# djordjijeK/DynamicGraphRepresentationLearning

Measured on AMD Instinct MI355X. Metric: MH walk-steps/sec, higher is better.
Workload: dtype u32

## Files before the change

dynamicgraphrepresentationlearning_amd/csrc/wharf_api.hip:

```cpp
#include <algorithm>
#include <cmath>
#include <cstring>

#include <rocprim/device/device_radix_sort.hpp>
#include <rocprim/device/device_scan.hpp>
#include <rocprim/device/device_segmented_radix_sort.hpp>
#include <rocprim/device/device_select.hpp>
#include <rocprim/iterator/counting_iterator.hpp>

#include <charconv>
#include <unistd.h>
#include <chrono>
#include <stdexcept>
#include <string>
#include <vector>

#include "wharf_gpu.h"
#include "wharf_kernels.h"

using namespace wharf;

namespace {

thread_local std::string g_last_error;
// ... 43 lines not shown
    }
    void release()
    {
        if (p) (void)hipFree(p);
        p = nullptr;
        cap = 0;
    }
    template <class T> T* as() const { return reinterpret_cast<T*>(p); }
};

uint32_t bits_for(uint64_t x)
{
    uint32_t b = 0;
    while (b < 64 && (x - 1) >> b) b++;
    return b;
}

}

struct wharf_handle {
    int device = 0;
    hipStream_t s = nullptr;
    hipEvent_t ev[6] = {};
    wharf_config cfg{};
    uint64_t n = 0, m = 0, lo = 0, hi = 0, n_loc = 0, W = 0;
    uint32_t sh_part = 0, sh_parts = 1, sh_bits = 0;

    ShardMap smap() const { return ShardMap{n, n_loc, lo, sh_part, sh_parts, sh_bits}; }
    bool owned_li(uint64_t wid, uint64_t& li) const
    {
        const uint64_t r = wid / n, v = wid % n;
        if (r >= wpv || v < lo || v >= hi) return false;
        const uint64_t off = v - lo, q = off >> sh_bits;
        if (q % sh_parts != sh_part) return false;
        li = r * n_loc + (((q / sh_parts) << sh_bits) | (off & ((1ull << sh_bits) - 1)));
        return true;
    }
    uint32_t L = 0, wpv = 0;
    bool anchors = false, has_walks = false;
    bool walks_poisoned = false;
    void check_walks() const
    {
        REQUIRE(!walks_poisoned, WHARF_E_STATE,
                "the walks are incomplete after a failed update (WHARF_E_STATE); call wharf_generate");
    }
    bool anchors_cold = true;
// ... 560 lines not shown
        a.ehash = anchors ? ehash.as<uint64_t>() : nullptr;
        a.ehash_mask = ehash_mask;
        a.fdir = anchors && fpool.p ? fdir.as<uint64_t>() : nullptr;
        a.fpool = anchors && fpool.p ? fpool.as<uint32_t>() : nullptr;
        a.walks = walks.as<uint32_t>();
        a.rtab = rtab.as<uint64_t>();
        a.bitmap = bitmap.as<uint32_t>();
        a.bloom = bitmap.as<uint32_t>() + bitmap_words();
        a.aff = aff.as<uint8_t>();
        a.counters = counters.as<unsigned long long>();
        a.n = n; a.n_loc = n_loc; a.lo = lo; a.W = W; a.wpv = wpv;
        a.sh_part = sh_part; a.sh_parts = sh_parts; a.sh_bits = sh_bits;
        a.L = L; a.epoch = epoch;
        a.key0 = (uint32_t)cfg.seed; a.key1 = (uint32_t)(cfg.seed >> 32);
        a.inv_p = 1.0f / cfg.paramP;
        a.inv_q = 1.0f / cfg.paramQ;
        a.model = cfg.model; a.init = cfg.sampler_init; a.det = cfg.deterministic;
        const char* ns = getenv("WHARF_NO_SURE_SKIP");
        a.no_sure = ns && atoi(ns) ? 1 : 0;
        const char* ls = getenv("WHARF_N2V_LANE_SORT");
        a.lane_sort = ls && *ls ? (atoi(ls) != 0) : 1;
        a.err = errflag.as<unsigned long long>() + 5;
        a.stage = 0;
        const char* rf = getenv("WHARF_RET_FIRST");
        a.ret_first = cfg.model == WHARF_NODE2VEC && !cfg.deterministic && cfg.sampler_init == WHARF_INIT_WEIGHT &&
                      !a.no_sure && a.inv_q != 1.0f && a.inv_p > fmaxf(1.0f, a.inv_q) && rf && *rf && atoi(rf) != 0;
        return a;
    }

    float elapsed(int a, int b)
    {
        float ms = 0;
        HIPCHK(hipEventElapsedTime(&ms, ev[a], ev[b]));
        return ms;
    }

    void read_counters()
    {
        unsigned long long c[8] = {};
        HIPCHK(hipMemcpyAsync(c, counters.p, 64, hipMemcpyDeviceToHost, s));
        sync();
        st.steps = c[0];
        st.accepts = c[1];
        st.last_anchor_inits = c[7];
        st.last_rewalk_passes = st_park_passes;
#ifdef WHARF_INIT_STATS
// ... 26 lines not shown
    try {
        if (h) HIPCHK(hipSetDevice(h->device));
        f();
        return WHARF_OK;
    } catch (const WharfError& e) {
        set_err(h, e.what());
        return e.code;
    } catch (const std::exception& e) {
        set_err(h, e.what());
        return WHARF_E_INVALID;
    }
}

void check_config(const wharf_config* c)
{
    REQUIRE(c, WHARF_E_INVALID, "config is null");
    REQUIRE(c->walks_per_vertex >= 1 && c->walks_per_vertex <= 255, WHARF_E_INVALID, "walks_per_vertex must be 1..255");
    REQUIRE(c->walk_length >= 2 && c->walk_length <= 255, WHARF_E_INVALID, "walk_length must be 2..255 (types::Position is u8)");
    REQUIRE(c->model == WHARF_DEEPWALK || c->model == WHARF_NODE2VEC, WHARF_E_INVALID, "Unrecognized random walking model");
    REQUIRE(c->sampler_init >= WHARF_INIT_RANDOM && c->sampler_init <= WHARF_INIT_WEIGHT, WHARF_E_INVALID,
            "Unrecognized sampler init strategy");
    REQUIRE(c->model != WHARF_NODE2VEC || (c->paramP > 0 && c->paramQ > 0), WHARF_E_INVALID, "paramP/paramQ must be > 0");
}

wharf_handle* new_handle(const wharf_config* cfg, uint64_t n, int device)
{
    check_config(cfg);
    REQUIRE(n >= 1 && n < 0xFFFFFFFEull, WHARF_E_INVALID, "n must be in [1, 2^32-2)");
    REQUIRE(n * (uint64_t)cfg->walks_per_vertex < (1ull << 32), WHARF_E_INVALID,
            "n * walks_per_vertex must be < 2^32 (types::WalkID is u32)");
    int ndev = 0;
    HIPCHK(hipGetDeviceCount(&ndev));
    REQUIRE(device >= 0 && device < ndev, WHARF_E_INVALID, "no such HIP device " + std::to_string(device));
    HIPCHK(hipSetDevice(device));
    auto* h = new wharf_handle();
    h->device = device;
    h->cfg = *cfg;
    h->n = n;
    h->L = cfg->walk_length;
    h->wpv = cfg->walks_per_vertex;
    h->lo = cfg->shard_lo;
    h->hi = cfg->shard_hi ? cfg->shard_hi : n;
    if (h->lo > h->hi || h->hi > n) {
        delete h;
        throw WharfError(WHARF_E_INVALID, "shard range must satisfy shard_lo <= shard_hi <= n");
    }
    h->n_loc = h->hi - h->lo;
    h->W = h->n_loc * h->wpv;
    h->anchors = cfg->model == WHARF_NODE2VEC && !cfg->deterministic;
    HIPCHK(hipStreamCreateWithFlags(&h->s, hipStreamNonBlocking));
    for (auto& e : h->ev) HIPCHK(hipEventCreate(&e));
    std::vector<uint64_t> t((size_t)h->wpv * h->L);
    for (uint32_t r = 0; r < h->wpv; r++) {
        XoroHost x(r);
        for (uint32_t j = 0; j < h->L; j++) t[(size_t)r * h->L + j] = x.lrand();
    }
    h->rtab.ensure(t.size() * 8);
    HIPCHK(hipMemcpy(h->rtab.p, t.data(), t.size() * 8, hipMemcpyHostToDevice));
    h->counters.ensure(64);
    h->errflag.ensure(64);
    return h;
}

void free_handle(wharf_handle* h)
{
    if (!h) return;
    (void)hipSetDevice(h->device);
    if (h->s) (void)hipStreamSynchronize(h->s);
    for (DevBuf* b : {&h->off, &h->adj, &h->deg, &h->cap, &h->vrec, &h->erec, &h->erec2, &h->ehash, &h->fdir, &h->fpool,
                      &h->fplan, &h->memo, &h->srcidx, &h->row_epoch, &h->off2, &h->adj2, &h->walks, &h->aff, &h->rtab,
                      &h->bitmap, &h->counters, &h->errflag, &h->tmp, &h->k1, &h->k2, &h->flags, &h->chg, &h->cf,
                      &h->runstart, &h->runs, &h->count, &h->pairs, &h->sel, &h->defer, &h->rplan, &h->pscan,
                      &h->scratch, &h->stab, &h->preoff, &h->park, &h->parkc, &h->bdesc, &h->sanc, &h->rchunk,
                      &h->rev, &h->srev, &h->sg_counts, &h->sg_noise, &h->sg_ids, &h->sg_cols, &h->sg_stat,
                      &h->sg_out})
        b->release();
    h->free_snaps();
    for (auto& e : h->ev)
        if (e) (void)hipEventDestroy(e);
    if (h->s) (void)hipStreamDestroy(h->s);
    delete h;
}

void build_graph_from_keys(wharf_handle* h, uint64_t cnt, bool drop_loops, bool symmetric_by_construction)
{
    const uint64_t mm = h->unique_keys(cnt, drop_loops, 32 + std::max<uint32_t>(bits_for(h->n), 1));
    h->symmetric = symmetric_by_construction;
    h->csr_from_keys(mm);
    const char* rv = getenv("WHARF_REV");
    const bool rev_may = rv && *rv ? atoi(rv) != 0 : h->pool_cap >= wharf_handle::kRevMinPool;
    if (!symmetric_by_construction && (h->anchors || rev_may)) {
        unsigned long long* asym = h->errflag.as<unsigned long long>() + 3;
        HIPCHK(hipMemsetAsync(asym, 0, 8, h->s));
        launch_keys_symmetric(h->k1.as<uint64_t>(), mm, asym, h->s);
        unsigned long long v = 1;
        HIPCHK(hipMemcpyAsync(&v, asym, 8, hipMemcpyDeviceToHost, h->s));
        h->sync();
        h->symmetric = v == 0;
    }
    for (DevBuf* b : {&h->k1, &h->k2, &h->tmp, &h->flags}) b->release();
    h->finish_graph();
}
// ... 28 lines not shown
    if (!listn) return;
    h->park.ensure(2 * listn * kParkRecBytes);
    h->parkc.ensure(16);
    unsigned long long* pc = h->parkc.as<unsigned long long>();
    char* P[2] = {h->park.as<char>(), h->park.as<char>() + listn * kParkRecBytes};
    HIPCHK(hipMemsetAsync(pc, 0, 16, s));
    launch_rewalk_park(a, 1, 1, nullptr, nullptr, P[0], pc, s);
    const char* te = getenv("WHARF_PARK_TAIL");
    const uint64_t tail = te ? strtoull(te, nullptr, 10) : kParkTail;
    uint32_t passes = 1;
    for (int cur = 0;; cur ^= 1) {
        uint64_t cnt = 0;
        HIPCHK(hipMemcpyAsync(&cnt, pc + cur, 8, hipMemcpyDeviceToHost, s));
        h->sync();
        if (!cnt) break;
        launch_park_init(a, P[cur], pc + cur, s);
        const bool last = cnt < tail;
        HIPCHK(hipMemsetAsync(pc + (cur ^ 1), 0, 8, s));
        launch_rewalk_park(a, 0, last ? 0 : 1, P[cur], pc + cur, P[cur ^ 1], pc + (cur ^ 1), s);
        passes++;
        if (last) break;
    }
    h->st_park_passes = passes;
}

void walk_update(wharf_handle* h, uint64_t k, uint32_t flags, uint32_t* affected_out, uint64_t* n_affected)
{
    hipStream_t s = h->s;
    if (h->has_walks && h->W) {
        HIPCHK(hipMemsetAsync(h->counters.p, 0, 24, s));
        HIPCHK(hipMemsetAsync(h->counters.as<unsigned long long>() + 7, 0, 8, s));
        h->st_park_passes = 0;
        const char* sat = getenv("WHARF_BLOOM_SATURATE");
        if (sat && atoi(sat)) HIPCHK(hipMemsetAsync(h->bitmap.as<uint32_t>() + h->bitmap_words(), 0xFF, kFilterWords * 4, s));
        WalkArgs a = h->walk_args();
        a.scan_only = (flags & WHARF_APPLY_WALK_UPDATES) ? 0 : 1;
        const char* ntr = getenv("WHARF_NT_ROWS");
        a.nt_rows = ntr ? (atoi(ntr) != 0) : ((double)k * h->L >= 0.08 * (double)std::max<uint64_t>(h->n, 1));
        const uint64_t stride4 = (h->L + 3) & ~3ull;
        const char* no_memo = getenv("WHARF_NO_MEMO");
        if (a.det && !a.scan_only && k && !(no_memo && atoi(no_memo)) &&
            (uint64_t)h->wpv * k * stride4 * 4 <= (256ull << 20)) {
            h->srcidx.ensure(std::max<uint64_t>(h->n, 1) * 4);
            h->memo.ensure(((uint64_t)h->wpv * k * stride4 + 2 * kMemoPad) * 4);
            const char* cbm = getenv("WHARF_COPY_BITMAP");
            a.src_exact = !(cbm && atoi(cbm));
// ... 55 lines not shown
        const bool corrupt = n2v_list && lbad && atoi(lbad) != 0;
        if (gsort || corrupt) {
            a.stage = 1;
            launch_walk(a, true, s);
            uint64_t c2 = 0;
            HIPCHK(hipMemcpyAsync(&c2, a.counters + 2, 8, hipMemcpyDeviceToHost, s));
            h->sync();
            const uint64_t cnt = c2 & kListMask;
            REQUIRE(cnt <= h->W, WHARF_E_STATE, "re-walk list longer than the walks");
            if (gsort && cnt > 1) {
                h->park.ensure(cnt * 8);
                uint64_t* in = h->defer.as<uint64_t>();
                uint64_t* out = h->park.as<uint64_t>();
                h->rp([&](void* t, size_t& b) { return rocprim::radix_sort_keys(t, b, in, out, (size_t)cnt, 0u, 64u, s); });
                HIPCHK(hipMemcpyAsync(in, out, cnt * 8, hipMemcpyDeviceToDevice, s));
            }
            if (corrupt && cnt) {
                const uint64_t bad = (h->W + 12345) | (1ull << 56);
                HIPCHK(hipMemcpyAsync(h->defer.as<uint64_t>() + cnt / 2, &bad, 8, hipMemcpyHostToDevice, s));
                h->sync();
            }
            a.stage = 2;
        }
        launch_walk(a, true, s);
        HIPCHK(hipGetLastError());
        if (a.park) park_passes(h, a);
        HIPCHK(hipEventRecord(h->ev[3], s));
        const unsigned nb = aff_blocks(h->W);
        h->sel.ensure((uint64_t)(nb + 1) * 8);
        uint32_t* bcount = h->sel.as<uint32_t>();
        uint32_t* boff = bcount + nb + 1;
        HIPCHK(hipMemsetAsync(bcount + nb, 0, 4, s));
        launch_aff_count(h->aff.as<uint8_t>(), h->W, bcount, s);
        h->rp([&](void* t, size_t& b) {
            return rocprim::exclusive_scan(t, b, bcount, boff, 0u, (size_t)nb + 1, rocprim::plus<uint32_t>(), s);
        });
        const bool on_device = affected_out && (flags & WHARF_AFFECTED_DEVICE);
        if (!on_device) h->pairs.ensure(h->W * 4);
        launch_aff_write(h->aff.as<uint8_t>(), h->W, boff, h->smap(),
                         on_device ? affected_out : h->pairs.as<uint32_t>(), s);
        uint32_t naff32 = 0;
        unsigned long long lerr = 0;
        HIPCHK(hipMemcpyAsync(&naff32, boff + nb, 4, hipMemcpyDeviceToHost, s));
        HIPCHK(hipMemcpyAsync(&lerr, a.err, 8, hipMemcpyDeviceToHost, s));
        h->sync();
        if (lerr) h->walks_poisoned = true;
        REQUIRE(lerr == 0, WHARF_E_STATE,
                std::string("node2vec re-walk list: ") + ((lerr & 1) ? "an entry outside the walks" : "an entry outside its block") +
                    " was skipped; the walks of this update are incomplete");
        const uint64_t naff = naff32;
        if (affected_out && !on_device && naff) {
            HIPCHK(hipMemcpyAsync(affected_out, h->pairs.p, naff * 4, hipMemcpyDeviceToHost, s));
            h->sync();
        }
        h->last_aff.clear();
        h->last_aff_version = ~0ull;
        if (!on_device && naff && naff <= wharf_handle::kStageMax) {
            if (affected_out) {
                h->last_aff.assign(affected_out, affected_out + naff);
            } else {
                h->last_aff.resize(naff);
                HIPCHK(hipMemcpyAsync(h->last_aff.data(), h->pairs.p, naff * 4, hipMemcpyDeviceToHost, s));
                h->sync();
            }
            h->last_aff_version = h->walks_version;
        }
        h->st.affected = naff;
        if (n_affected) *n_affected = naff;
        h->read_counters();
        h->st.last_walk_kernel_ms = h->elapsed(2, 3);
        h->st.last_walk_update_ms = h->elapsed(1, 3);
    } else {
        h->sync();
    }
// ... 1158 lines not shown
```

dynamicgraphrepresentationlearning_amd/csrc/wharf_kernels.h:

```cpp
#pragma once

#include <hip/hip_runtime.h>
#include <stdint.h>

#include <algorithm>

#include "wharf_device.h"

namespace wharf {

enum { kDeepWalk = 0, kNode2Vec = 1 };
enum { kInitRandom = 0, kInitBurnin = 1, kInitWeight = 2 };
constexpr uint64_t kMemoPad = 64;

struct RunInfo {
    uint64_t off, end;
    uint32_t src, rs, re, pad;
};

struct WalkArgs {
    const ERec* vrec;
    const ERec* erec;
    RecFmt rf;
    const uint32_t* deg;
// ... 15 lines not shown
    uint32_t key0, key1;
    float inv_p, inv_q;
    int model, init, det;
    int scan_only;
    uint64_t* defer;
    uint64_t* bdesc;
    uint64_t* stab;
    uint64_t stab_mask;
    uint32_t* memo;
    const uint32_t* src_idx;
    const RunInfo* runs;
    uint64_t memo_k;
    uint32_t memo_stride;
    uint32_t wpv;
    int nt_rows;
    int park;
    int no_sure;
    int lane_sort;
    int src_exact;
    int ret_first;
    unsigned long long* err;
    int stage;
    int plan_group;
};

__host__ __device__ __forceinline__ ShardMap shard_map(const WalkArgs& a)
{
    return ShardMap{a.n, a.n_loc, a.lo, a.sh_part, a.sh_parts, a.sh_bits};
}

constexpr uint64_t kListMask = (1ull << 40) - 1;
constexpr uint64_t kParkRecBytes = 32;


constexpr uint64_t kRelocate = ~0ull;
struct RowPlan {
    uint64_t noff;
    uint32_t ndeg, ncap;
    uint32_t ocap, pad;
};

unsigned grid_for(uint64_t work, unsigned block);
unsigned cu_count();

void launch_walk(const WalkArgs& a, bool rewalk, hipStream_t s);
void launch_rewalk_park(const WalkArgs& a, int fresh, int park, const void* in, const unsigned long long* in_cnt,
// ... 64 lines not shown
                      hipStream_t s);
void launch_patch_in_edges(const uint32_t* adj, uint64_t slots, const uint32_t* bitmap, const uint32_t* bloom,
                           const ERec* vrec, ERec* erec, uint32_t rs, RecFmt rf, hipStream_t s);
constexpr uint32_t kNoRidx = 0xFFFFFFFFu;
void launch_rev_build(const uint64_t* off, const uint32_t* deg, const uint32_t* adj, uint64_t n, uint64_t slots,
                      uint32_t* ridx, unsigned long long* miss, hipStream_t s);
void launch_patch_rev(const RunInfo* runs, uint64_t k, const uint32_t* pre, const uint64_t* off, const uint32_t* deg,
                      const uint32_t* adj, const uint32_t* bitmap, const ERec* vrec, ERec* erec, uint32_t rs,
                      RecFmt rf, uint32_t* ridx, unsigned long long* miss, hipStream_t s);
void launch_transpose(const uint32_t* in, uint64_t W, uint32_t L, uint32_t* out, hipStream_t s);
void launch_gather_rows(const uint32_t* walks, uint64_t W, uint32_t L, const uint64_t* list, uint64_t base,
                        uint64_t count, uint32_t* out, hipStream_t s);
void launch_walk_lengths(const uint32_t* walks, uint64_t W, uint32_t L, uint32_t v0, uint32_t v1, uint64_t* len,
                         hipStream_t s);
void launch_index_entries(const uint32_t* walks, uint64_t W, uint32_t L, const ShardMap& sm, int kb,
                          uint32_t v0, uint32_t v1, const uint64_t* col_base, uint64_t* skeys, uint32_t* vals,
                          hipStream_t s);
void launch_index_split(const uint64_t* skeys, uint64_t E, int kb, unsigned long long* counts, uint64_t* keys,
                        hipStream_t s);
unsigned aff_blocks(uint64_t W);
void launch_aff_count(const uint8_t* aff, uint64_t W, uint32_t* counts, hipStream_t s);
void launch_aff_write(const uint8_t* aff, uint64_t W, const uint32_t* offs, const ShardMap& sm,
                      uint32_t* out, hipStream_t s);
void launch_index_pair(const uint64_t* keys, const uint32_t* nexts, uint64_t E, uint64_t* out, hipStream_t s);
void launch_rel_offsets(const uint64_t* off, uint64_t v0, uint64_t cnt, uint32_t* rel, hipStream_t s);
void launch_fill_u32(uint32_t* p, uint64_t cnt, uint32_t v, hipStream_t s);
void launch_fill_u64(uint64_t* p, uint64_t cnt, uint64_t v, hipStream_t s);
void launch_edge_hash_update(const uint64_t* bkeys, uint64_t mb, const uint32_t* chg, int insert, uint64_t* table,
                             uint64_t mask, hipStream_t s);
void launch_edge_hash_build(const uint64_t* off, const uint32_t* deg, uint64_t n, const uint32_t* adj, uint64_t* table,
                            uint64_t mask, hipStream_t s);
void launch_filter_sizes(const uint32_t* deg, uint64_t n, uint64_t* words, hipStream_t s);
void launch_filter_pack(const uint32_t* deg, uint64_t n, uint64_t* fdir, hipStream_t s);
void launch_filter_fill(const uint64_t* off, const uint32_t* deg, uint64_t n, const uint32_t* adj, const uint64_t* fdir,
                        uint32_t* pool, hipStream_t s);
void launch_filter_plan(const RunInfo* runs, uint64_t k, const uint32_t* deg, const uint64_t* fdir, uint64_t* need,
                        hipStream_t s);
void launch_filter_rows(const RunInfo* runs, uint64_t k, const uint32_t* pre, const uint64_t* noff, const uint32_t* deg,
                        const uint32_t* adj, const uint64_t* need, const uint64_t* gofs, uint64_t base, uint64_t* fdir,
                        uint32_t* pool, hipStream_t s);
void launch_szudzik64(int op, uint64_t cnt, uint64_t* x, uint64_t* y, uint64_t* z, hipStream_t s);

constexpr uint32_t kSgnsNone = 0xFFFFFFFFu;
constexpr uint32_t kSgnsMaxTargets = 16;
constexpr uint32_t kSgnsMaxWindow = 16;
constexpr uint64_t kSgnsSerialCap = 1ull << 20;
// ... 23 lines not shown
```

dynamicgraphrepresentationlearning_amd/csrc/wharf_kernels.hip:

```cpp
#include <cstdlib>
#include <string>
#include <type_traits>

#include "wharf_kernels.h"

namespace wharf {

__device__ __forceinline__ void wave_add(unsigned long long* dst, uint32_t v)
{
#pragma unroll
    for (int o = 32; o > 0; o >>= 1) v += __shfl_xor(v, o, 64);
    if ((threadIdx.x & 63) == 0 && v) atomicAdd(dst, (unsigned long long)v);
}

__device__ __forceinline__ int64_t row_find(const uint32_t* __restrict__ adj, const Row& r, uint32_t x)
{
    uint64_t lo = r.off, hi = r.off + r.deg;
    while (lo < hi) {
        const uint64_t mid = lo + ((hi - lo) >> 1);
        if (adj[mid] < x) lo = mid + 1; else hi = mid;
    }
    return (lo < r.off + r.deg && adj[lo] == x) ? (int64_t)lo : -1;
}

// ... 647 lines not shown
            steps++;
        }
        for (pos = pos + 1; pos < a.L; pos++) walks[(uint64_t)pos * W + li] = kSent;
    }
    wave_add(a.counters + 0, steps);
    wave_add(a.counters + 1, accepts);
    wave_add(a.counters + 7, inits);
}

enum : uint32_t { kLaneScan = 0, kLaneWalk = 1, kLaneDone = 2 };

__device__ __forceinline__ void bloom_to_lds(const WalkArgs& a, uint32_t* s_bloom)
{
    for (uint32_t i = threadIdx.x; i < kBloomWords; i += blockDim.x) s_bloom[i] = a.bloom[i];
    __syncthreads();
}

__device__ __forceinline__ bool is_source(const WalkArgs& a, const uint32_t* s_bloom, uint32_t x)
{
    if (!bloom_test(s_bloom, x)) return false;
    return (a.bitmap[x >> 5] >> (x & 31)) & 1u;
}

template <int MODEL, bool DET, bool BLK = false, int RL = -1>
__global__ __launch_bounds__(256) void k_rewalk_sweep(WalkArgs a)
{
    __shared__ uint32_t s_bloom[kBloomWords];
    bloom_to_lds(a, s_bloom);
    uint32_t steps = 0, accepts = 0, inits = 0;
    const uint64_t stride = (uint64_t)gridDim.x * blockDim.x;
    uint32_t* __restrict__ walks = a.walks;
    const uint64_t W = a.W;
    const uint32_t L = a.L;
    for (uint64_t li = (uint64_t)blockIdx.x * blockDim.x + threadIdx.x; li < W; li += stride) {
        const uint64_t r = li / a.n_loc;
        const uint32_t v = BLK ? walks[li] : start_vertex<false>(a, li - r * a.n_loc);
        const uint64_t wid = r * a.n + v;
        const uint32_t ep = a.epoch << 4, wlo = (uint32_t)wid, whi = (uint32_t)(wid >> 32);
        const uint64_t* __restrict__ rt = DET ? a.rtab + r * L : nullptr;
        uint32_t mode = kLaneScan, p = kNoRewalk;
        uint32_t x = v, xprev = v;
        uint32_t xn = L > 1 ? walks[W + li] : kSent;
        Walker w;
        w.rc.deg = 0;
        for (uint32_t pos = 0; pos < L; pos++) {
            uint32_t val = kSent;
            bool fresh = false;
            if (mode == kLaneWalk) {
                if (w.rc.deg) {
                    val = walk_step<MODEL, DET, false, false, RL>(a, w, rt, DET ? pos - 1 - p : pos - 1, wlo, whi, ep,
                                                                  accepts, inits);
                    steps++;
                }
                fresh = true;
            } else if (mode == kLaneScan) {
                if (pos > 0) {
                    xprev = x;
// ... 186 lines not shown
        if ((a.bitmap[v >> 5] >> (v & 31)) & 1u) return j;
    }
#endif
    ended = t.end < cnt;
    return kScanChunk;
}

__device__ __forceinline__ uint64_t uniform64(uint64_t x)
{
    const uint32_t lo = __builtin_amdgcn_readfirstlane((uint32_t)x), hi = __builtin_amdgcn_readfirstlane((uint32_t)(x >> 32));
    return ((uint64_t)hi << 32) | lo;
}

struct XcdRange {
    uint64_t first, end, stride;
};
__device__ __forceinline__ XcdRange xcd_range(uint64_t W)
{
    const uint32_t xcd = blockIdx.x % kXcds, slot = blockIdx.x / kXcds, per = gridDim.x / kXcds;
    const uint64_t part = (((W + kXcds - 1) / kXcds) + 255) & ~255ull;
    const uint64_t c0 = min(W, (uint64_t)xcd * part);
    return {c0 + (uint64_t)slot * blockDim.x + threadIdx.x, min(W, c0 + part), (uint64_t)per * blockDim.x};
}

#ifndef WHARF_SCAN_WAVES_EU
#define WHARF_SCAN_WAVES_EU 0
#endif
#if WHARF_SCAN_WAVES_EU
#define WHARF_SCAN_WAVES __attribute__((amdgpu_waves_per_eu(WHARF_SCAN_WAVES_EU, WHARF_SCAN_WAVES_EU)))
#else
#define WHARF_SCAN_WAVES
#endif

#ifndef WHARF_SCAN_ONLY_WAVES_EU
#define WHARF_SCAN_ONLY_WAVES_EU 8
#endif
#ifndef WHARF_COPY_EARLY_ROWS
#define WHARF_COPY_EARLY_ROWS 0
#endif
#ifndef WHARF_COPY_WAVES
#define WHARF_COPY_WAVES 1
#endif
template <bool COPY, bool NTL, int FB = 0, bool IDX = false>
__global__ __launch_bounds__(256, COPY ? WHARF_COPY_WAVES : WHARF_SCAN_ONLY_WAVES_EU) WHARF_SCAN_WAVES void k_rewalk_chunked(WalkArgs a)
{
    constexpr uint32_t C = kScanChunk;
    __shared__ uint32_t s_bloom[kBloomWords << FB];
    filter_to_lds<FB>(a, s_bloom);
    uint32_t steps = 0;
    uint32_t* __restrict__ walks = a.walks;
    const uint64_t W = a.W;
    const uint32_t L = a.L;
    const XcdRange xr = xcd_range(W);
    const uint32_t lane = __lane_id();
    for (uint64_t li = xr.first; li < xr.end; li += xr.stride) {
        const uint64_t r = li / a.n_loc;
        uint32_t p = kNoRewalk;
        bool scanning = true;
        const uint32_t* __restrict__ row = nullptr;
        uint32_t* __restrict__ wb = walks + uniform64(li - lane);
        uint32_t cur[C], nxt[C];
#pragma unroll
        for (uint32_t j = 0; j < C; j++) cur[j] = j < L ? row_load<NTL>(wb + (uint64_t)j * W, lane) : kSent;
        for (uint32_t c0 = 0; c0 < L; c0 += C) {
            const uint32_t cnt = min(C, L - c0);
            const bool was_scanning = scanning;
            const bool more = c0 + C < L;
            ChunkTest ct;
            if (scanning) chunk_issue<FB, WHARF_CHUNK_LEAN != 0, COPY && IDX>(a, s_bloom, cur, cnt, ct);
            if ((!COPY || WHARF_COPY_EARLY_ROWS) && more && scanning) {
#pragma unroll
                for (uint32_t j = 0; j < C; j++)
                    nxt[j] = c0 + C + j < L ? row_load<NTL>(wb + (uint64_t)(c0 + C + j) * W, lane) : kSent;
            }
            if (scanning) {
                bool ended = false;
// ... 717 lines not shown
static unsigned walk_grid(uint64_t W)
{
    static int per_cu = -1;
    if (per_cu < 0) {
        const char* e = getenv("WHARF_WALK_BLOCKS_PER_CU");
        per_cu = e ? std::max(0, atoi(e)) : 0;
    }
    const uint64_t full = (W + 255) / 256;
    if (per_cu <= 0) return (unsigned)full;
    return (unsigned)std::min<uint64_t>(full, (uint64_t)cu_count() * per_cu);
}

static unsigned list_grid() { return cu_count() * 8; }

static bool flat_list()
{
    const char* e = getenv("WHARF_N2V_REWALK");
    return e && std::string(e) == "flat";
}

void launch_walk(const WalkArgs& a, bool rewalk, hipStream_t s)
{
    if (a.W == 0) return;
    const dim3 grid(rewalk ? std::min<uint64_t>((a.W + 255) / 256, (uint64_t)cu_count() * 8) : walk_grid(a.W)),
        block(256);
    const dim3 lgrid(list_grid());
    const char* pk = getenv("WHARF_PLAN_KERNEL");
    const bool plan_lean = !(pk && std::string(pk) == "chunked") && a.W <= kLeanMaxW;
    const dim3 pgrid((unsigned)std::min<uint64_t>((a.W + 1023) / 1024, (uint64_t)cu_count() * 2));
    const dim3 bgrid((std::max<unsigned>(std::min<uint64_t>((a.W + 1023) / 1024, (uint64_t)cu_count() * 2), kXcds) /
                      kXcds) * kXcds);
    const char* ps = getenv("WHARF_PLAN_SPLIT");
    const bool plan_split = ps && *ps && atoi(ps) != 0;
    const bool cr = a.rf.compact != 0;
#define WHARF_LAUNCH(M, D)                                                                   \
    do {                                                                                     \
        if (rewalk && M == kNode2Vec) {                                                      \
            if (a.stage == 2) {                                                              \
            } else if (plan_lean && plan_split) {                                            \
                if (a.nt_rows) hipLaunchKernelGGL((k_rewalk_scan_lean<true>), bgrid, dim3(1024), 0, s, a); \
                else hipLaunchKernelGGL((k_rewalk_scan_lean<false>), bgrid, dim3(1024), 0, s, a); \
                hipLaunchKernelGGL((k_rewalk_plan_lean<false, true>), pgrid, dim3(1024), 0, s, a); \
            } else if (plan_lean) {                                                          \
                if (a.nt_rows) hipLaunchKernelGGL(k_rewalk_plan_lean<true>, pgrid, dim3(1024), 0, s, a); \
                else hipLaunchKernelGGL(k_rewalk_plan_lean<false>, pgrid, dim3(1024), 0, s, a);  \
            } else {                                                                         \
                hipLaunchKernelGGL(k_rewalk_plan, grid, block, 0, s, a);                     \
            }                                                                                \
              \
            if (!a.scan_only && !a.park && a.stage != 1) {                                   \
                if (a.bdesc) hipLaunchKernelGGL((k_rewalk_block<M>), lgrid, block, 0, s, a);     \
                else if (flat_list()) hipLaunchKernelGGL((k_rewalk_list<M, D>), lgrid, block, 0, s, a); \
                else if (a.ret_first) hipLaunchKernelGGL((k_rewalk_sorted<M, D, M == kNode2Vec>), lgrid, block, 0, s, a); \
                else hipLaunchKernelGGL((k_rewalk_sorted<M, D>), lgrid, block, 0, s, a);     \
            }                                                                                \
        } else if (rewalk) {                                                                 \
            if (cr && a.sh_parts > 1) hipLaunchKernelGGL((k_rewalk_sweep<M, D, true, 1>), grid, block, 0, s, a); \
            else if (cr) hipLaunchKernelGGL((k_rewalk_sweep<M, D, false, 1>), grid, block, 0, s, a); \
            else if (a.sh_parts > 1) hipLaunchKernelGGL((k_rewalk_sweep<M, D, true, 0>), grid, block, 0, s, a); \
            else hipLaunchKernelGGL((k_rewalk_sweep<M, D, false, 0>), grid, block, 0, s, a);     \
        } else {                                                                             \
            if (cr && a.sh_parts > 1) hipLaunchKernelGGL((k_walk<M, D, true, 1>), grid, block, 0, s, a); \
            else if (cr) hipLaunchKernelGGL((k_walk<M, D, false, 1>), grid, block, 0, s, a); \
            else if (a.sh_parts > 1) hipLaunchKernelGGL((k_walk<M, D, true, 0>), grid, block, 0, s, a); \
            else hipLaunchKernelGGL((k_walk<M, D, false, 0>), grid, block, 0, s, a);         \
        }                                                                                    \
    } while (0)
    const dim3 mgrid((std::max<unsigned>(grid.x, kXcds) / kXcds) * kXcds);
    const char* nc = getenv("WHARF_NO_CHUNKED_SCAN");
    const bool chunked = !(nc && atoi(nc));
    if (rewalk && a.det && a.memo && !a.scan_only) {
        hipLaunchKernelGGL(k_det_suffix, grid_for((uint64_t)a.wpv * a.memo_k, 256), 256, 0, s, a);
        const char* cb = getenv("WHARF_COPY_SMALL_BLOOM");
        if (cb && atoi(cb) && a.src_exact) {
            if (a.nt_rows) hipLaunchKernelGGL((k_rewalk_chunked<true, true, 0, true>), mgrid, block, 0, s, a);
            else hipLaunchKernelGGL((k_rewalk_chunked<true, false, 0, true>), mgrid, block, 0, s, a);
        } else if (cb && atoi(cb)) {
            if (a.nt_rows) hipLaunchKernelGGL((k_rewalk_chunked<true, true, 0>), mgrid, block, 0, s, a);
            else hipLaunchKernelGGL((k_rewalk_chunked<true, false, 0>), mgrid, block, 0, s, a);
        } else if (a.src_exact) {
            if (a.nt_rows) hipLaunchKernelGGL((k_rewalk_chunked<true, true, 1, true>), mgrid, block, 0, s, a);
            else hipLaunchKernelGGL((k_rewalk_chunked<true, false, 1, true>), mgrid, block, 0, s, a);
        } else {
            if (a.nt_rows) hipLaunchKernelGGL((k_rewalk_chunked<true, true, 1>), mgrid, block, 0, s, a);
            else hipLaunchKernelGGL((k_rewalk_chunked<true, false, 1>), mgrid, block, 0, s, a);
        }
        return;
    }
    if (rewalk && a.scan_only && chunked) {
        const char* sb = getenv("WHARF_SCAN_SMALL_BLOOM");
        const char* sk = getenv("WHARF_SCAN_KERNEL");
        const bool small = sb && atoi(sb), big = sk && std::string(sk) == "big";
        if (!small && !big && a.W <= kLeanMaxW) {
            if (a.nt_rows) hipLaunchKernelGGL((k_rewalk_scan_lean<true>), bgrid, dim3(1024), 0, s, a);
            else hipLaunchKernelGGL((k_rewalk_scan_lean<false>), bgrid, dim3(1024), 0, s, a);
            return;
        }
        if (!small) {
            if (a.nt_rows) hipLaunchKernelGGL((k_rewalk_scan_big<true>), bgrid, dim3(1024), 0, s, a);
            else hipLaunchKernelGGL((k_rewalk_scan_big<false>), bgrid, dim3(1024), 0, s, a);
            return;
        }
        if (a.nt_rows) hipLaunchKernelGGL((k_rewalk_chunked<false, true>), mgrid, block, 0, s, a);
        else hipLaunchKernelGGL((k_rewalk_chunked<false, false>), mgrid, block, 0, s, a);
        return;
    }
    if (a.det) WHARF_LAUNCH(kDeepWalk, true);
    else if (a.model == kDeepWalk) WHARF_LAUNCH(kDeepWalk, false);
    else WHARF_LAUNCH(kNode2Vec, false);
// ... 926 lines not shown
        keys[i] = k & mask;
        atomicAdd(counts + (k >> kb), 1ull);
    }
}

constexpr uint32_t kAffPerThread = 16, kAffPerBlock = 256 * kAffPerThread;

__device__ __forceinline__ uint32_t aff_count16(const uint8_t* __restrict__ aff, uint64_t W, uint64_t base)
{
    uint32_t c = 0;
    if (base + kAffPerThread <= W) {
        const uint4 q = *reinterpret_cast<const uint4*>(aff + base);
        const uint32_t w[4] = {q.x, q.y, q.z, q.w};
#pragma unroll
        for (int k = 0; k < 4; k++)
#pragma unroll
            for (int b = 0; b < 4; b++) c += ((w[k] >> (8 * b)) & 0xFFu) != kNoRewalk;
    } else {
        for (uint64_t i = base; i < W; i++) c += aff[i] != kNoRewalk;
    }
    return c;
}

__global__ __launch_bounds__(256) void k_aff_count(const uint8_t* __restrict__ aff, uint64_t W, uint32_t* __restrict__ counts)
{
    const uint64_t base = (uint64_t)blockIdx.x * kAffPerBlock + (uint64_t)threadIdx.x * kAffPerThread;
    uint32_t c = base < W ? aff_count16(aff, W, base) : 0;
#pragma unroll
    for (int o = 32; o > 0; o >>= 1) c += __shfl_xor(c, o, 64);
    __shared__ uint32_t part[4];
    if ((threadIdx.x & 63) == 0) part[threadIdx.x >> 6] = c;
    __syncthreads();
    if (threadIdx.x == 0) counts[blockIdx.x] = part[0] + part[1] + part[2] + part[3];
}

__global__ __launch_bounds__(256) void k_aff_write(const uint8_t* __restrict__ aff, uint64_t W, const uint32_t* __restrict__ offs,
                                                   ShardMap sm, uint32_t* __restrict__ out)
{
    const uint64_t base = (uint64_t)blockIdx.x * kAffPerBlock + (uint64_t)threadIdx.x * kAffPerThread;
    const uint32_t c = base < W ? aff_count16(aff, W, base) : 0;
    const uint32_t lane = threadIdx.x & 63, wv = threadIdx.x >> 6;
    uint32_t x = c;
#pragma unroll
    for (int o = 1; o < 64; o <<= 1) {
        const uint32_t y = __shfl_up(x, o, 64);
        if (lane >= (uint32_t)o) x += y;
    }
    __shared__ uint32_t part[4];
    if (lane == 63) part[wv] = x;
    __syncthreads();
    uint32_t pre = x - c;
    for (uint32_t k = 0; k < wv; k++) pre += part[k];
    uint64_t at = (uint64_t)offs[blockIdx.x] + pre;
    if (!c) return;
    const uint64_t end = base + kAffPerThread < W ? base + kAffPerThread : W;
    for (uint64_t l = base; l < end; l++) {
        if (aff[l] == kNoRewalk) continue;
        out[at++] = (uint32_t)sm.wid(l);
    }
}

unsigned aff_blocks(uint64_t W) { return (unsigned)((W + kAffPerBlock - 1) / kAffPerBlock); }
void launch_aff_count(const uint8_t* aff, uint64_t W, uint32_t* counts, hipStream_t s)
{ if (W) hipLaunchKernelGGL(k_aff_count, aff_blocks(W), 256, 0, s, aff, W, counts); }
void launch_aff_write(const uint8_t* aff, uint64_t W, const uint32_t* offs, const ShardMap& sm, uint32_t* out,
                      hipStream_t s)
{ if (W) hipLaunchKernelGGL(k_aff_write, aff_blocks(W), 256, 0, s, aff, W, offs, sm, out); }

__global__ void k_fill_u64(uint64_t* __restrict__ p, uint64_t cnt, uint64_t v)
{
    for (uint64_t i = (uint64_t)blockIdx.x * blockDim.x + threadIdx.x; i < cnt; i += (uint64_t)gridDim.x * blockDim.x)
        p[i] = v;
}

__global__ void k_fill_u32(uint32_t* __restrict__ p, uint64_t cnt, uint32_t v)
{
    for (uint64_t i = (uint64_t)blockIdx.x * blockDim.x + threadIdx.x; i < cnt; i += (uint64_t)gridDim.x * blockDim.x)
        p[i] = v;
}

__device__ __forceinline__ uint64_t isqrt64(uint64_t z)
{
    uint64_t s = (uint64_t)sqrt((double)z);
    while (s * s > z) s--;
    while ((s + 1) * (s + 1) <= z && (s + 1) < 0x100000000ull) s++;
    return s;
}

__global__ void k_szudzik64(int op, uint64_t cnt, uint64_t* __restrict__ x, uint64_t* __restrict__ y, uint64_t* __restrict__ z)
{
// ... 241 lines not shown
```

dynamicgraphrepresentationlearning_amd/distributed.py:

```python
from __future__ import annotations

import os
from dataclasses import dataclass

import numpy as np


class RankFailure(RuntimeError):

    def __init__(self, rank: int, phase: str, message: str):
        super().__init__(f"rank {rank} failed in {phase}: {message}")
        self.rank = rank
        self.phase = phase
        self.message = message


def _dist_active(group=None) -> bool:
    import torch.distributed as dist
    return dist.is_available() and dist.is_initialized()


def agree(err, phase: str, group=None, device="cpu"):
    if not _dist_active(group):
        if err is not None:
# ... 246 lines not shown

    total = torch.zeros((), dtype=torch.int64, device=rows.device)
    pos = torch.arange(L, dtype=torch.int64, device=rows.device)
    for r0 in range(0, rows.shape[0], block_rows):
        blk = rows[r0:r0 + block_rows]
        ids = torch.arange(global_first + r0, global_first + r0 + blk.shape[0], dtype=torch.int64, device=rows.device)
        h = (ids[:, None] * L + pos[None, :]) * _K1
        h = (h ^ (h >> 31)) * _K2
        total += (((blk.to(torch.int64) & 0xFFFFFFFF) + 1) * h).sum()
    return total


def local_corpus_checksum(read_local, shard, n: int, wpv: int, L: int, rows_per_call: int, device="cpu"):
    import torch

    own = shard_size(shard) * wpv
    buf = torch.empty((max(1, min(rows_per_call, own)), L), dtype=torch.int32, device=device)
    total = torch.zeros((), dtype=torch.int64, device=device)
    for f in range(0, own, buf.shape[0]):
        k = min(buf.shape[0], own - f)
        read_local(f, k, buf[:k])
        for lf, c, gf in shard_rows_to_global(shard, n, f, k):
            total += corpus_checksum(buf[lf - f:lf - f + c], gf, L)
    return total
```

Measured before the change: 50.56 billion.

## Slice walk update to overlap affected-id D2H copies with re-walking

```diff
diff --git a/dynamicgraphrepresentationlearning_amd/csrc/wharf_api.hip b/dynamicgraphrepresentationlearning_amd/csrc/wharf_api.hip
--- a/dynamicgraphrepresentationlearning_amd/csrc/wharf_api.hip
+++ b/dynamicgraphrepresentationlearning_amd/csrc/wharf_api.hip
@@ -89,6 +89,10 @@
     int device = 0;
     hipStream_t s = nullptr;
     hipEvent_t ev[6] = {};
+    static constexpr uint32_t kMaxAffSlices = 64;
+    hipStream_t s2 = nullptr;
+    hipEvent_t sev[kMaxAffSlices] = {};
+    uint32_t* slice_cnt = nullptr;
     wharf_config cfg{};
     uint64_t n = 0, m = 0, lo = 0, hi = 0, n_loc = 0, W = 0;
     uint32_t sh_part = 0, sh_parts = 1, sh_bits = 0;
@@ -695,6 +699,7 @@
         a.lane_sort = ls && *ls ? (atoi(ls) != 0) : 1;
         a.err = errflag.as<unsigned long long>() + 5;
         a.stage = 0;
+        a.w_first = 0; a.w_end = W;
         const char* rf = getenv("WHARF_RET_FIRST");
         a.ret_first = cfg.model == WHARF_NODE2VEC && !cfg.deterministic && cfg.sampler_init == WHARF_INIT_WEIGHT &&
                       !a.no_sure && a.inv_q != 1.0f && a.inv_p > fmaxf(1.0f, a.inv_q) && rf && *rf && atoi(rf) != 0;
@@ -767,6 +772,8 @@
             "Unrecognized sampler init strategy");
     REQUIRE(c->model != WHARF_NODE2VEC || (c->paramP > 0 && c->paramQ > 0), WHARF_E_INVALID, "paramP/paramQ must be > 0");
 }
+
+void free_handle(wharf_handle* h);
 
 wharf_handle* new_handle(const wharf_config* cfg, uint64_t n, int device)
 {
@@ -793,17 +800,25 @@
     h->n_loc = h->hi - h->lo;
     h->W = h->n_loc * h->wpv;
     h->anchors = cfg->model == WHARF_NODE2VEC && !cfg->deterministic;
-    HIPCHK(hipStreamCreateWithFlags(&h->s, hipStreamNonBlocking));
-    for (auto& e : h->ev) HIPCHK(hipEventCreate(&e));
-    std::vector<uint64_t> t((size_t)h->wpv * h->L);
-    for (uint32_t r = 0; r < h->wpv; r++) {
-        XoroHost x(r);
-        for (uint32_t j = 0; j < h->L; j++) t[(size_t)r * h->L + j] = x.lrand();
-    }
-    h->rtab.ensure(t.size() * 8);
-    HIPCHK(hipMemcpy(h->rtab.p, t.data(), t.size() * 8, hipMemcpyHostToDevice));
-    h->counters.ensure(64);
-    h->errflag.ensure(64);
+    try {
+        HIPCHK(hipStreamCreateWithFlags(&h->s, hipStreamNonBlocking));
+        for (auto& e : h->ev) HIPCHK(hipEventCreate(&e));
+        HIPCHK(hipStreamCreateWithFlags(&h->s2, hipStreamNonBlocking));
+        for (auto& e : h->sev) HIPCHK(hipEventCreateWithFlags(&e, hipEventDisableTiming));
+        HIPCHK(hipHostMalloc((void**)&h->slice_cnt, wharf_handle::kMaxAffSlices * sizeof(uint32_t), hipHostMallocDefault));
+        std::vector<uint64_t> t((size_t)h->wpv * h->L);
+        for (uint32_t r = 0; r < h->wpv; r++) {
+            XoroHost x(r);
+            for (uint32_t j = 0; j < h->L; j++) t[(size_t)r * h->L + j] = x.lrand();
+        }
+        h->rtab.ensure(t.size() * 8);
+        HIPCHK(hipMemcpy(h->rtab.p, t.data(), t.size() * 8, hipMemcpyHostToDevice));
+        h->counters.ensure(64);
+        h->errflag.ensure(64);
+    } catch (...) {
+        free_handle(h);
+        throw;
+    }
     return h;
 }
 
@@ -812,6 +827,7 @@
     if (!h) return;
     (void)hipSetDevice(h->device);
     if (h->s) (void)hipStreamSynchronize(h->s);
+    if (h->s2) (void)hipStreamSynchronize(h->s2);
     for (DevBuf* b : {&h->off, &h->adj, &h->deg, &h->cap, &h->vrec, &h->erec, &h->erec2, &h->ehash, &h->fdir, &h->fpool,
                       &h->fplan, &h->memo, &h->srcidx, &h->row_epoch, &h->off2, &h->adj2, &h->walks, &h->aff, &h->rtab,
                       &h->bitmap, &h->counters, &h->errflag, &h->tmp, &h->k1, &h->k2, &h->flags, &h->chg, &h->cf,
@@ -823,6 +839,10 @@
     h->free_snaps();
     for (auto& e : h->ev)
         if (e) (void)hipEventDestroy(e);
+    for (auto& e : h->sev)
+        if (e) (void)hipEventDestroy(e);
+    if (h->slice_cnt) (void)hipHostFree(h->slice_cnt);
+    if (h->s2) (void)hipStreamDestroy(h->s2);
     if (h->s) (void)hipStreamDestroy(h->s);
     delete h;
 }
@@ -897,6 +917,85 @@
         if (last) break;
     }
     h->st_park_passes = passes;
+}
+
+constexpr uint64_t kAffSlicesDefault = 8;
+constexpr uint64_t kSliceRounds = 4;
+
+uint64_t slice_blocks(const wharf_handle* h, const WalkArgs& a, uint32_t flags, const uint32_t* affected_out)
+{
+    if (!affected_out || (flags & WHARF_AFFECTED_DEVICE) || a.scan_only) return 0;
+    if (!a.det && a.model != kDeepWalk) return 0;
+    const char* ks = getenv("WHARF_AFF_SLICES");
+    uint64_t K = ks && *ks ? strtoull(ks, nullptr, 10) : kAffSlicesDefault;
+    K = std::min<uint64_t>(K, wharf_handle::kMaxAffSlices);
+    uint64_t min_walks = kSliceRounds * cu_count() * 8 * 256;
+    const char* mw = getenv("WHARF_AFF_SLICE_MIN_WALKS");
+    if (mw && *mw) min_walks = std::max<uint64_t>(strtoull(mw, nullptr, 10), 1);
+    const uint64_t blocks = (h->W + 255) / 256;
+    K = std::min(K, std::min(blocks, h->W / min_walks));
+    if (K < 2) return 0;
+    hipPointerAttribute_t at{};
+    if (hipPointerGetAttributes(&at, affected_out) != hipSuccess) {
+        (void)hipGetLastError();
+        return 0;
+    }
+    if (at.type != hipMemoryTypeHost) return 0;
+    return (blocks + K - 1) / K;
+}
+
+uint64_t walk_update_sliced(wharf_handle* h, WalkArgs a, uint64_t per_blocks, uint32_t* affected_out)
+{
+    hipStream_t s = h->s, s2 = h->s2;
+    const uint64_t W = h->W, per = per_blocks * 256, nsl = (W + per - 1) / per;
+    REQUIRE(nsl <= wharf_handle::kMaxAffSlices, WHARF_E_STATE, "too many slices of the walks");
+    const char* lg = getenv("WHARF_LOG_SLICES");
+    if (lg && atoi(lg))
+        fprintf(stderr, "[wharf] walk update: %llu slices of %llu walks\n", (unsigned long long)nsl, (unsigned long long)per);
+    const uint64_t slot = (uint64_t)aff_blocks(per) + 1;
+    h->sel.ensure(nsl * slot * 8);
+    h->pairs.ensure(W * 4);
+    uint32_t* sel = h->sel.as<uint32_t>();
+    uint32_t* ids = h->pairs.as<uint32_t>();
+    uint64_t naff = 0;
+    try {
+        HIPCHK(hipMemsetAsync(sel, 0, nsl * slot * 8, s));
+        for (uint64_t k = 0; k < nsl; k++) {
+            a.w_first = k * per;
+            a.w_end = std::min(W, a.w_first + per);
+            launch_walk(a, true, s);
+            if (k + 1 == nsl) {
+                HIPCHK(hipGetLastError());
+                HIPCHK(hipEventRecord(h->ev[3], s));
+            }
+            const unsigned nb = aff_blocks(a.w_end - a.w_first);
+            uint32_t* bcount = sel + 2 * k * slot;
+            uint32_t* boff = bcount + slot;
+            launch_aff_count(h->aff.as<uint8_t>(), a.w_first, a.w_end, bcount, s);
+            h->rp([&](void* t, size_t& b) {
+                return rocprim::exclusive_scan(t, b, bcount, boff, 0u, (size_t)nb + 1, rocprim::plus<uint32_t>(), s);
+            });
+            launch_aff_write(h->aff.as<uint8_t>(), a.w_first, a.w_end, boff, h->smap(), ids + a.w_first, s);
+            HIPCHK(hipEventRecord(h->sev[k], s));
+        }
+        for (uint64_t k = 0; k < nsl; k++) {
+            const uint64_t first = k * per, end = std::min(W, first + per);
+            const uint32_t* boff = sel + 2 * k * slot + slot;
+            HIPCHK(hipStreamWaitEvent(s2, h->sev[k], 0));
+            HIPCHK(hipMemcpyAsync(h->slice_cnt + k, boff + aff_blocks(end - first), 4, hipMemcpyDeviceToHost, s2));
+            HIPCHK(hipStreamSynchronize(s2));
+            const uint64_t cnt = h->slice_cnt[k];
+            REQUIRE(cnt <= end - first, WHARF_E_STATE, "affected-id count of a slice exceeds its walks");
+            if (cnt) HIPCHK(hipMemcpyAsync(affected_out + naff, ids + first, cnt * 4, hipMemcpyDeviceToHost, s2));
+            naff += cnt;
+        }
+        HIPCHK(hipStreamSynchronize(s2));
+    } catch (...) {
+        (void)hipStreamSynchronize(s2);
+        (void)hipStreamSynchronize(s);
+        throw;
+    }
+    return naff;
 }
 
 void walk_update(wharf_handle* h, uint64_t k, uint32_t flags, uint32_t* affected_out, uint64_t* n_affected)
@@ -998,34 +1097,42 @@
             }
             a.stage = 2;
         }
-        launch_walk(a, true, s);
-        HIPCHK(hipGetLastError());
-        if (a.park) park_passes(h, a);
-        HIPCHK(hipEventRecord(h->ev[3], s));
-        const unsigned nb = aff_blocks(h->W);
-        h->sel.ensure((uint64_t)(nb + 1) * 8);
-        uint32_t* bcount = h->sel.as<uint32_t>();
-        uint32_t* boff = bcount + nb + 1;
-        HIPCHK(hipMemsetAsync(bcount + nb, 0, 4, s));
-        launch_aff_count(h->aff.as<uint8_t>(), h->W, bcount, s);
-        h->rp([&](void* t, size_t& b) {
-            return rocprim::exclusive_scan(t, b, bcount, boff, 0u, (size_t)nb + 1, rocprim::plus<uint32_t>(), s);
-        });
         const bool on_device = affected_out && (flags & WHARF_AFFECTED_DEVICE);
-        if (!on_device) h->pairs.ensure(h->W * 4);
-        launch_aff_write(h->aff.as<uint8_t>(), h->W, boff, h->smap(),
-                         on_device ? affected_out : h->pairs.as<uint32_t>(), s);
-        uint32_t naff32 = 0;
+        const uint64_t slice = slice_blocks(h, a, flags, affected_out);
+        uint64_t naff = 0;
         unsigned long long lerr = 0;
-        HIPCHK(hipMemcpyAsync(&naff32, boff + nb, 4, hipMemcpyDeviceToHost, s));
-        HIPCHK(hipMemcpyAsync(&lerr, a.err, 8, hipMemcpyDeviceToHost, s));
-        h->sync();
+        if (slice) {
+            naff = walk_update_sliced(h, a, slice, affected_out);
+            HIPCHK(hipMemcpyAsync(&lerr, a.err, 8, hipMemcpyDeviceToHost, s));
+            h->sync();
+        } else {
+            launch_walk(a, true, s);
+            HIPCHK(hipGetLastError());
+            if (a.park) park_passes(h, a);
+            HIPCHK(hipEventRecord(h->ev[3], s));
+            const unsigned nb = aff_blocks(h->W);
+            h->sel.ensure((uint64_t)(nb + 1) * 8);
+            uint32_t* bcount = h->sel.as<uint32_t>();
+            uint32_t* boff = bcount + nb + 1;
+            HIPCHK(hipMemsetAsync(bcount + nb, 0, 4, s));
+            launch_aff_count(h->aff.as<uint8_t>(), h->W, bcount, s);
+            h->rp([&](void* t, size_t& b) {
+                return rocprim::exclusive_scan(t, b, bcount, boff, 0u, (size_t)nb + 1, rocprim::plus<uint32_t>(), s);
+            });
+            if (!on_device) h->pairs.ensure(h->W * 4);
+            launch_aff_write(h->aff.as<uint8_t>(), h->W, boff, h->smap(),
+                             on_device ? affected_out : h->pairs.as<uint32_t>(), s);
+            uint32_t naff32 = 0;
+            HIPCHK(hipMemcpyAsync(&naff32, boff + nb, 4, hipMemcpyDeviceToHost, s));
+            HIPCHK(hipMemcpyAsync(&lerr, a.err, 8, hipMemcpyDeviceToHost, s));
+            h->sync();
+            naff = naff32;
+        }
         if (lerr) h->walks_poisoned = true;
         REQUIRE(lerr == 0, WHARF_E_STATE,
                 std::string("node2vec re-walk list: ") + ((lerr & 1) ? "an entry outside the walks" : "an entry outside its block") +
                     " was skipped; the walks of this update are incomplete");
-        const uint64_t naff = naff32;
-        if (affected_out && !on_device && naff) {
+        if (!slice && affected_out && !on_device && naff) {
             HIPCHK(hipMemcpyAsync(affected_out, h->pairs.p, naff * 4, hipMemcpyDeviceToHost, s));
             h->sync();
         }
diff --git a/dynamicgraphrepresentationlearning_amd/csrc/wharf_kernels.h b/dynamicgraphrepresentationlearning_amd/csrc/wharf_kernels.h
--- a/dynamicgraphrepresentationlearning_amd/csrc/wharf_kernels.h
+++ b/dynamicgraphrepresentationlearning_amd/csrc/wharf_kernels.h
@@ -61,6 +61,7 @@
     unsigned long long* err;
     int stage;
     int plan_group;
+    uint64_t w_first, w_end;
 };
 
 __host__ __device__ __forceinline__ ShardMap shard_map(const WalkArgs& a)
@@ -171,6 +172,9 @@
 void launch_aff_count(const uint8_t* aff, uint64_t W, uint32_t* counts, hipStream_t s);
 void launch_aff_write(const uint8_t* aff, uint64_t W, const uint32_t* offs, const ShardMap& sm,
                       uint32_t* out, hipStream_t s);
+void launch_aff_count(const uint8_t* aff, uint64_t first, uint64_t end, uint32_t* counts, hipStream_t s);
+void launch_aff_write(const uint8_t* aff, uint64_t first, uint64_t end, const uint32_t* offs, const ShardMap& sm,
+                      uint32_t* out, hipStream_t s);
 void launch_index_pair(const uint64_t* keys, const uint32_t* nexts, uint64_t E, uint64_t* out, hipStream_t s);
 void launch_rel_offsets(const uint64_t* off, uint64_t v0, uint64_t cnt, uint32_t* rel, hipStream_t s);
 void launch_fill_u32(uint32_t* p, uint64_t cnt, uint32_t v, hipStream_t s);
diff --git a/dynamicgraphrepresentationlearning_amd/csrc/wharf_kernels.hip b/dynamicgraphrepresentationlearning_amd/csrc/wharf_kernels.hip
--- a/dynamicgraphrepresentationlearning_amd/csrc/wharf_kernels.hip
+++ b/dynamicgraphrepresentationlearning_amd/csrc/wharf_kernels.hip
@@ -693,7 +693,7 @@
     return (a.bitmap[x >> 5] >> (x & 31)) & 1u;
 }
 
-template <int MODEL, bool DET, bool BLK = false, int RL = -1>
+template <int MODEL, bool DET, bool BLK = false, int RL = -1, bool RANGE = false>
 __global__ __launch_bounds__(256) void k_rewalk_sweep(WalkArgs a)
 {
     __shared__ uint32_t s_bloom[kBloomWords];
@@ -703,7 +703,8 @@
     uint32_t* __restrict__ walks = a.walks;
     const uint64_t W = a.W;
     const uint32_t L = a.L;
-    for (uint64_t li = (uint64_t)blockIdx.x * blockDim.x + threadIdx.x; li < W; li += stride) {
+    const uint64_t w0 = RANGE ? a.w_first : 0, w1 = RANGE ? a.w_end : W;
+    for (uint64_t li = w0 + (uint64_t)blockIdx.x * blockDim.x + threadIdx.x; li < w1; li += stride) {
         const uint64_t r = li / a.n_loc;
         const uint32_t v = BLK ? walks[li] : start_vertex<false>(a, li - r * a.n_loc);
         const uint64_t wid = r * a.n + v;
@@ -936,6 +937,13 @@
     const uint64_t c0 = min(W, (uint64_t)xcd * part);
     return {c0 + (uint64_t)slot * blockDim.x + threadIdx.x, min(W, c0 + part), (uint64_t)per * blockDim.x};
 }
+__device__ __forceinline__ XcdRange xcd_range(uint64_t first, uint64_t end)
+{
+    const uint32_t xcd = blockIdx.x % kXcds, slot = blockIdx.x / kXcds, per = gridDim.x / kXcds;
+    const uint64_t part = (((end - first + kXcds - 1) / kXcds) + 255) & ~255ull;
+    const uint64_t c0 = min(end, first + (uint64_t)xcd * part);
+    return {c0 + (uint64_t)slot * blockDim.x + threadIdx.x, min(end, c0 + part), (uint64_t)per * blockDim.x};
+}
 
 #ifndef WHARF_SCAN_WAVES_EU
 #define WHARF_SCAN_WAVES_EU 0
@@ -955,7 +963,7 @@
 #ifndef WHARF_COPY_WAVES
 #define WHARF_COPY_WAVES 1
 #endif
-template <bool COPY, bool NTL, int FB = 0, bool IDX = false>
+template <bool COPY, bool NTL, int FB = 0, bool IDX = false, bool RANGE = false>
 __global__ __launch_bounds__(256, COPY ? WHARF_COPY_WAVES : WHARF_SCAN_ONLY_WAVES_EU) WHARF_SCAN_WAVES void k_rewalk_chunked(WalkArgs a)
 {
     constexpr uint32_t C = kScanChunk;
@@ -965,7 +973,7 @@
     uint32_t* __restrict__ walks = a.walks;
     const uint64_t W = a.W;
     const uint32_t L = a.L;
-    const XcdRange xr = xcd_range(W);
+    const XcdRange xr = (COPY && RANGE) ? xcd_range(a.w_first, a.w_end) : xcd_range(W);
     const uint32_t lane = __lane_id();
     for (uint64_t li = xr.first; li < xr.end; li += xr.stride) {
         const uint64_t r = li / a.n_loc;
@@ -1729,7 +1737,10 @@
 void launch_walk(const WalkArgs& a, bool rewalk, hipStream_t s)
 {
     if (a.W == 0) return;
-    const dim3 grid(rewalk ? std::min<uint64_t>((a.W + 255) / 256, (uint64_t)cu_count() * 8) : walk_grid(a.W)),
+    const uint64_t span = a.w_end > a.w_first ? a.w_end - a.w_first : 0;
+    if (rewalk && span == 0) return;
+    const bool ranged = rewalk && span != a.W;
+    const dim3 grid(rewalk ? std::min<uint64_t>((span + 255) / 256, (uint64_t)cu_count() * 8) : walk_grid(a.W)),
         block(256);
     const dim3 lgrid(list_grid());
     const char* pk = getenv("WHARF_PLAN_KERNEL");
@@ -1761,6 +1772,11 @@
                 else if (a.ret_first) hipLaunchKernelGGL((k_rewalk_sorted<M, D, M == kNode2Vec>), lgrid, block, 0, s, a); \
                 else hipLaunchKernelGGL((k_rewalk_sorted<M, D>), lgrid, block, 0, s, a);     \
             }                                                                                \
+        } else if (rewalk && ranged) {        \
+            if (cr && a.sh_parts > 1) hipLaunchKernelGGL((k_rewalk_sweep<kDeepWalk, D, true, 1, true>), grid, block, 0, s, a); \
+            else if (cr) hipLaunchKernelGGL((k_rewalk_sweep<kDeepWalk, D, false, 1, true>), grid, block, 0, s, a); \
+            else if (a.sh_parts > 1) hipLaunchKernelGGL((k_rewalk_sweep<kDeepWalk, D, true, 0, true>), grid, block, 0, s, a); \
+            else hipLaunchKernelGGL((k_rewalk_sweep<kDeepWalk, D, false, 0, true>), grid, block, 0, s, a); \
         } else if (rewalk) {                                                                 \
             if (cr && a.sh_parts > 1) hipLaunchKernelGGL((k_rewalk_sweep<M, D, true, 1>), grid, block, 0, s, a); \
             else if (cr) hipLaunchKernelGGL((k_rewalk_sweep<M, D, false, 1>), grid, block, 0, s, a); \
@@ -1777,21 +1793,26 @@
     const char* nc = getenv("WHARF_NO_CHUNKED_SCAN");
     const bool chunked = !(nc && atoi(nc));
     if (rewalk && a.det && a.memo && !a.scan_only) {
-        hipLaunchKernelGGL(k_det_suffix, grid_for((uint64_t)a.wpv * a.memo_k, 256), 256, 0, s, a);
+        if (a.w_first == 0) hipLaunchKernelGGL(k_det_suffix, grid_for((uint64_t)a.wpv * a.memo_k, 256), 256, 0, s, a);
         const char* cb = getenv("WHARF_COPY_SMALL_BLOOM");
-        if (cb && atoi(cb) && a.src_exact) {
-            if (a.nt_rows) hipLaunchKernelGGL((k_rewalk_chunked<true, true, 0, true>), mgrid, block, 0, s, a);
-            else hipLaunchKernelGGL((k_rewalk_chunked<true, false, 0, true>), mgrid, block, 0, s, a);
-        } else if (cb && atoi(cb)) {
-            if (a.nt_rows) hipLaunchKernelGGL((k_rewalk_chunked<true, true, 0>), mgrid, block, 0, s, a);
-            else hipLaunchKernelGGL((k_rewalk_chunked<true, false, 0>), mgrid, block, 0, s, a);
-        } else if (a.src_exact) {
-            if (a.nt_rows) hipLaunchKernelGGL((k_rewalk_chunked<true, true, 1, true>), mgrid, block, 0, s, a);
-            else hipLaunchKernelGGL((k_rewalk_chunked<true, false, 1, true>), mgrid, block, 0, s, a);
+        const int fb = cb && atoi(cb) ? 0 : 1;
+#define WHARF_COPY(FB, IDX, RANGE)                                                                       \
+    do {                                                                                                 \
+        if (a.nt_rows) hipLaunchKernelGGL((k_rewalk_chunked<true, true, FB, IDX, RANGE>), mgrid, block, 0, s, a); \
+        else hipLaunchKernelGGL((k_rewalk_chunked<true, false, FB, IDX, RANGE>), mgrid, block, 0, s, a);  \
+    } while (0)
+        if (ranged) {
+            if (fb == 0 && a.src_exact) WHARF_COPY(0, true, true);
+            else if (fb == 0) WHARF_COPY(0, false, true);
+            else if (a.src_exact) WHARF_COPY(1, true, true);
+            else WHARF_COPY(1, false, true);
         } else {
-            if (a.nt_rows) hipLaunchKernelGGL((k_rewalk_chunked<true, true, 1>), mgrid, block, 0, s, a);
-            else hipLaunchKernelGGL((k_rewalk_chunked<true, false, 1>), mgrid, block, 0, s, a);
-        }
+            if (fb == 0 && a.src_exact) WHARF_COPY(0, true, false);
+            else if (fb == 0) WHARF_COPY(0, false, false);
+            else if (a.src_exact) WHARF_COPY(1, true, false);
+            else WHARF_COPY(1, false, false);
+        }
+#undef WHARF_COPY
         return;
     }
     if (rewalk && a.scan_only && chunked) {
@@ -2764,9 +2785,10 @@
     return c;
 }
 
-__global__ __launch_bounds__(256) void k_aff_count(const uint8_t* __restrict__ aff, uint64_t W, uint32_t* __restrict__ counts)
-{
-    const uint64_t base = (uint64_t)blockIdx.x * kAffPerBlock + (uint64_t)threadIdx.x * kAffPerThread;
+__global__ __launch_bounds__(256) void k_aff_count(const uint8_t* __restrict__ aff, uint64_t first, uint64_t W,
+                                                   uint32_t* __restrict__ counts)
+{
+    const uint64_t base = first + (uint64_t)blockIdx.x * kAffPerBlock + (uint64_t)threadIdx.x * kAffPerThread;
     uint32_t c = base < W ? aff_count16(aff, W, base) : 0;
 #pragma unroll
     for (int o = 32; o > 0; o >>= 1) c += __shfl_xor(c, o, 64);
@@ -2776,10 +2798,10 @@
     if (threadIdx.x == 0) counts[blockIdx.x] = part[0] + part[1] + part[2] + part[3];
 }
 
-__global__ __launch_bounds__(256) void k_aff_write(const uint8_t* __restrict__ aff, uint64_t W, const uint32_t* __restrict__ offs,
-                                                   ShardMap sm, uint32_t* __restrict__ out)
-{
-    const uint64_t base = (uint64_t)blockIdx.x * kAffPerBlock + (uint64_t)threadIdx.x * kAffPerThread;
+__global__ __launch_bounds__(256) void k_aff_write(const uint8_t* __restrict__ aff, uint64_t first, uint64_t W,
+                                                   const uint32_t* __restrict__ offs, ShardMap sm, uint32_t* __restrict__ out)
+{
+    const uint64_t base = first + (uint64_t)blockIdx.x * kAffPerBlock + (uint64_t)threadIdx.x * kAffPerThread;
     const uint32_t c = base < W ? aff_count16(aff, W, base) : 0;
     const uint32_t lane = threadIdx.x & 63, wv = threadIdx.x >> 6;
     uint32_t x = c;
@@ -2803,11 +2825,16 @@
 }
 
 unsigned aff_blocks(uint64_t W) { return (unsigned)((W + kAffPerBlock - 1) / kAffPerBlock); }
+void launch_aff_count(const uint8_t* aff, uint64_t first, uint64_t end, uint32_t* counts, hipStream_t s)
+{ if (end > first) hipLaunchKernelGGL(k_aff_count, aff_blocks(end - first), 256, 0, s, aff, first, end, counts); }
+void launch_aff_write(const uint8_t* aff, uint64_t first, uint64_t end, const uint32_t* offs, const ShardMap& sm,
+                      uint32_t* out, hipStream_t s)
+{ if (end > first) hipLaunchKernelGGL(k_aff_write, aff_blocks(end - first), 256, 0, s, aff, first, end, offs, sm, out); }
 void launch_aff_count(const uint8_t* aff, uint64_t W, uint32_t* counts, hipStream_t s)
-{ if (W) hipLaunchKernelGGL(k_aff_count, aff_blocks(W), 256, 0, s, aff, W, counts); }
+{ launch_aff_count(aff, 0, W, counts, s); }
 void launch_aff_write(const uint8_t* aff, uint64_t W, const uint32_t* offs, const ShardMap& sm, uint32_t* out,
                       hipStream_t s)
-{ if (W) hipLaunchKernelGGL(k_aff_write, aff_blocks(W), 256, 0, s, aff, W, offs, sm, out); }
+{ launch_aff_write(aff, 0, W, offs, sm, out, s); }
 
 __global__ void k_fill_u64(uint64_t* __restrict__ p, uint64_t cnt, uint64_t v)
 {
diff --git a/dynamicgraphrepresentationlearning_amd/distributed.py b/dynamicgraphrepresentationlearning_amd/distributed.py
--- a/dynamicgraphrepresentationlearning_amd/distributed.py
+++ b/dynamicgraphrepresentationlearning_amd/distributed.py
@@ -292,4 +292,6 @@
         read_local(f, k, buf[:k])
         for lf, c, gf in shard_rows_to_global(shard, n, f, k):
             total += corpus_checksum(buf[lf - f:lf - f + c], gf, L)
+        if buf.is_cuda:
+            torch.cuda.current_stream(buf.device).synchronize()
     return total
```

Result: slower. 49.80 billion (-1.5%).
